# Hamedkiri/heuristique_style_transfer_code

Hardware: NVIDIA B200
Metric: images/sec (higher is better)
Workload: dtype tf32

## Files before the change

### heuristique_style_transfer_code_b200/_lib.py

```python
from __future__ import annotations

import ctypes
import os
from ctypes import c_int, c_longlong, c_void_p, POINTER, c_uint

from .build import LIB_PATH

_LIB = None

GH_DTYPE_F32 = 0
GH_DTYPE_BF16 = 1
GH_ERR_BAD_ARG = -1
GH_ERR_UNSUPPORTED = -2

_P = c_void_p
_SIGNATURES = {
    "gh_version": (c_int, []),
    "gh_sm_count": (c_int, []),
    "gh_set_option": (c_int, [ctypes.c_char_p, c_int]),
    "gh_last_device_error": (c_int, [POINTER(c_uint)]),
    "gh_gram_pool_fwd": (c_int, [_P, c_int, c_longlong, c_longlong, c_longlong, c_int, c_int, c_int, c_int, _P, c_int,
                                  c_int, c_int, c_int, _P]),
    "gh_gram_dense_fwd": (c_int, [_P, c_int, c_longlong, c_longlong, c_longlong, c_int, c_int, c_int, _P, c_int, c_int,
                                   _P]),
    "gh_adaptive_pool_fwd": (c_int, [_P, c_int, c_int, c_int, _P, c_int, c_int, _P]),
    "gh_adaptive_pool_bwd": (c_int, [_P, c_int, c_int, c_int, c_int, c_int, _P, _P]),
    "gh_gram_pool_bwd": (c_int, [_P, c_int, c_longlong, c_longlong, c_longlong, c_int, c_int, c_int, c_int, _P, c_int,
                                  c_int, _P, c_int, c_longlong, c_longlong, c_longlong, c_int, _P]),
    "gh_gram_dense_bwd": (c_int, [_P, c_int, c_longlong, c_longlong, c_longlong, c_int, c_int, c_int, _P, _P, c_int,
                                   c_longlong, c_longlong, c_longlong, c_int, _P]),
    "gh_attn_head_fwd": (c_int, [_P] * 7 + [c_int] * 4 + [_P] * 5 + [_P]),
    "gh_transpose_cast": (c_int, [_P, c_int, _P, c_int, c_int, c_int, c_int, c_longlong, _P]),
    "gh_preprocess_frame": (c_int, [_P, c_longlong, c_int, c_int, c_int, _P, _P, _P, c_int, _P, _P, _P, c_int, _P, _P, _P,
                                     c_int, c_int, _P]),
    "gh_normalize_u8": (c_int, [_P, _P, c_longlong, c_int, c_longlong, _P, _P, _P]),
    "gh_gemm_f32": (c_int, [_P, c_longlong, c_longlong, _P, c_longlong, c_longlong, _P, _P, c_longlong, c_int, c_int,
                             c_int, _P]),
    "gh_maxpool2d_nhwc": (c_int, [_P, c_int, _P] + [c_int] * 7 + [_P]),
    "gh_stem_space_to_depth": (c_int, [_P] + [c_longlong] * 4 + [c_int] * 3 + [_P, c_int, _P]),
    "gh_patch_gram_workspace": (c_longlong, [c_int, c_int, c_int]),
    "gh_patch_gram_fwd": (c_int, [_P, _P, _P, _P, c_int, c_int, c_int, c_int, _P, _P, _P, _P]),
    "gh_patch_attn_fwd": (c_int, [_P] * 11 + [c_int] * 5 + [_P, _P, _P]),
    "gh_attn_head_bwd_workspace": (c_longlong, [c_int, c_int, c_int]),
    "gh_attn_head_bwd": (c_int, [_P] * 10 + [c_int] * 4 + [_P] * 8 + [_P]),
    "gh_gram_mse_blocks": (c_int, [c_longlong]),
    "gh_gram_mse": (c_int, [_P, _P, c_longlong, _P, _P, _P]),
    "gh_split_bf16": (c_int, [_P, _P, c_longlong, c_longlong, _P]),
    "gh_gemm_planes": (c_int, [_P, c_longlong, c_longlong, c_int, _P, c_longlong, c_longlong, c_int, _P, _P, _P,
                                c_longlong, c_longlong, c_int, c_int, c_int, c_int, _P]),
    "gh_tgemm_plan": (c_int, [c_int, c_int, c_int, c_int, c_int, POINTER(c_int), POINTER(c_int), POINTER(c_int)]),
    "gh_gram_bwd_plan": (c_int, [c_int, c_int, c_int, c_int, c_int, POINTER(c_int)]),
    "gh_attn_head_fwd2": (c_int, [_P] * 7 + [c_int] * 4 + [_P] * 6 + [_P]),
    "gh_attn_head_bwd2_workspace": (c_longlong, [c_int, c_int, c_int]),
    "gh_attn_head_bwd2": (c_int, [_P] * 10 + [c_int] * 4 + [_P] * 8 + [_P]),
}
EXPORTED_SYMBOLS = tuple(_SIGNATURES)


class GramHeadError(RuntimeError):
    pass


def library_path() -> str:
    return os.environ.get("GRAMHEAD_LIB", LIB_PATH)


def lib() -> ctypes.CDLL:
    global _LIB
    if _LIB is None:
        path = library_path()
        if not os.path.isfile(path):
            raise GramHeadError(
# ... 43 lines not shown
```

### heuristique_style_transfer_code_b200/build.py

```python
from __future__ import annotations

import os
import shutil
import subprocess

CSRC = os.path.join(os.path.dirname(os.path.abspath(__file__)), "csrc")
LIB_PATH = os.path.join(CSRC, "libgramhead.so")
SOURCES = ["gramhead.cu", "common.cuh", "gram_fwd.cuh", "pair.cuh", "gram_fwd_pair.cuh", "gram_bwd.cuh", "gram_bwd2.cuh", "gram_bwd_pair.cuh",
           "umma_gemm.cuh", "tgemm_pair.cuh", "launch.cuh", "attn_head.cuh", "attn_head2.cuh", "preprocess.cuh", "transpose.cuh", "patchgan.cuh", "pool.cuh", "style_loss.cuh"]
NVCC_FLAGS = ["-gencode", "arch=compute_100a,code=sm_100a", "-O3", "-lineinfo", "-std=c++17",
              "-Xcompiler", "-fPIC", "-shared"]


def _nvcc() -> str:
    for cand in (os.environ.get("NVCC"), shutil.which("nvcc"), "/usr/local/cuda/bin/nvcc"):
        if cand and os.path.isfile(cand):
            return cand
    raise RuntimeError("gramhead: nvcc not found (set NVCC=/path/to/nvcc)")


def is_stale() -> bool:
    if not os.path.isfile(LIB_PATH):
        return True
    built = os.path.getmtime(LIB_PATH)
    deps = [os.path.join(CSRC, s) for s in SOURCES]
    deps.append(os.path.join(os.path.dirname(os.path.dirname(CSRC)), "include", "gramhead.h"))
    return any(os.path.getmtime(d) > built for d in deps if os.path.isfile(d))


def build_library(force: bool = False, verbose: bool = False) -> str:
    if not force and not is_stale():
        return LIB_PATH
    cmd = [_nvcc(), *NVCC_FLAGS, "gramhead.cu", "-o", LIB_PATH + ".tmp"]
    if verbose:
        cmd.insert(1, "-Xptxas=-v")
    res = subprocess.run(cmd, cwd=CSRC, capture_output=True, text=True)
    if res.returncode != 0:
        raise RuntimeError("gramhead: nvcc failed\n" + res.stdout + res.stderr)
    if verbose:
        print(res.stderr)
    os.replace(LIB_PATH + ".tmp", LIB_PATH)
    return LIB_PATH
# ... 5 lines not shown
```

### heuristique_style_transfer_code_b200/csrc/common.cuh

```cuda
#pragma once
#include <cuda_runtime.h>
#include <cuda_bf16.h>
#include <stdint.h>

namespace gh {

__device__ unsigned int* g_dev_error_ptr = nullptr;

__device__ __forceinline__ void dev_fail(unsigned int code, unsigned int site) {
  unsigned int* rec = g_dev_error_ptr;
  if (rec != nullptr && atomicCAS_system(rec, 0u, code) == 0u) {
    rec[1] = blockIdx.x;
    rec[2] = threadIdx.x;
    rec[3] = site;
    __threadfence_system();
  }
  __trap();
}

inline volatile unsigned int* error_record_host() {
  static unsigned int* host_rec[64] = {nullptr};
  int dev = 0;
  if (cudaGetDevice(&dev) != cudaSuccess || dev < 0 || dev >= 64) return nullptr;
  if (host_rec[dev] == nullptr) {
// ... 130 lines not shown
      "{%0, %1, %2, %3, %4, %5, %6, %7, %8, %9, %10, %11, %12, %13, %14, %15, "
      "%16, %17, %18, %19, %20, %21, %22, %23, %24, %25, %26, %27, %28, %29, %30, %31}, [%32];"
      : "=r"(r[0]), "=r"(r[1]), "=r"(r[2]), "=r"(r[3]), "=r"(r[4]), "=r"(r[5]), "=r"(r[6]), "=r"(r[7]),
        "=r"(r[8]), "=r"(r[9]), "=r"(r[10]), "=r"(r[11]), "=r"(r[12]), "=r"(r[13]), "=r"(r[14]), "=r"(r[15]),
        "=r"(r[16]), "=r"(r[17]), "=r"(r[18]), "=r"(r[19]), "=r"(r[20]), "=r"(r[21]), "=r"(r[22]), "=r"(r[23]),
        "=r"(r[24]), "=r"(r[25]), "=r"(r[26]), "=r"(r[27]), "=r"(r[28]), "=r"(r[29]), "=r"(r[30]), "=r"(r[31])
      : "r"(taddr)
      : "memory");
}
__device__ __forceinline__ void tmem_ld_wait() { asm volatile("tcgen05.wait::ld.sync.aligned;" ::: "memory"); }

constexpr uint32_t kTileK = 64;
constexpr uint32_t kRowBytes = 128;
constexpr uint32_t kAtomBytes = 1024;
constexpr uint32_t kUmmaK = 16;

__host__ __device__ constexpr uint64_t make_smem_desc_sw128(uint32_t smem_addr) {
  return (uint64_t)((smem_addr & 0x3FFFFu) >> 4)
         | ((uint64_t)1 << 16)
         | ((uint64_t)(kAtomBytes >> 4) << 32)
         | ((uint64_t)1 << 46)
         | ((uint64_t)2 << 61);
}
__host__ __device__ constexpr uint32_t make_idesc_bf16(uint32_t m, uint32_t n) {
  return (1u << 4)
         | (1u << 7)
         | (1u << 10)
         | ((n >> 3) << 17)
         | ((m >> 4) << 24);
}
__device__ __forceinline__ uint32_t sw128_off(uint32_t r, uint32_t k) {
  return (r >> 3) * kAtomBytes + (r & 7u) * kRowBytes + ((((k >> 3) ^ r) & 7u) << 4) + ((k & 7u) << 1);
}

__device__ __forceinline__ float4 ldg_stream_f4(const float* p) {
  float4 v;
  asm volatile("ld.global.nc.L1::no_allocate.L2::128B.v4.f32 {%0, %1, %2, %3}, [%4];"
               : "=f"(v.x), "=f"(v.y), "=f"(v.z), "=f"(v.w)
               : "l"(p));
  return v;
}
__device__ __forceinline__ uint2 ldg_stream_u2(const void* p) {
  uint2 v;
  asm volatile("ld.global.nc.L1::no_allocate.v2.u32 {%0, %1}, [%2];" : "=r"(v.x), "=r"(v.y) : "l"(p));
  return v;
}
__device__ __forceinline__ void sts_u2(uint32_t addr, uint32_t a, uint32_t b) {
  asm volatile("st.shared.v2.b32 [%0], {%1, %2};" ::"r"(addr), "r"(a), "r"(b) : "memory");
}
__device__ __forceinline__ void sts_u4(uint32_t addr, uint32_t a, uint32_t b, uint32_t c, uint32_t d) {
  asm volatile("st.shared.v4.b32 [%0], {%1, %2, %3, %4};" ::"r"(addr), "r"(a), "r"(b), "r"(c), "r"(d) : "memory");
}
__device__ __forceinline__ uint32_t pack_bf16x2(float lo, float hi) {
  __nv_bfloat162 h = __floats2bfloat162_rn(lo, hi);
  return *reinterpret_cast<uint32_t*>(&h);
}
__device__ __forceinline__ void red_add_f32(float* p, float v) {
  asm volatile("red.global.add.f32 [%0], %1;" ::"l"(p), "f"(v) : "memory");
}

}
```

### heuristique_style_transfer_code_b200/csrc/gramhead.cu

```cuda
#include "../../include/gramhead.h"
#include "common.cuh"
#include "gram_fwd.cuh"
#include "gram_fwd_pair.cuh"
#include "gram_bwd.cuh"
#include "gram_bwd2.cuh"
#include "gram_bwd_pair.cuh"
#include "attn_head.cuh"
#include "umma_gemm.cuh"
#include "tgemm_pair.cuh"
#include "attn_head2.cuh"
#include "preprocess.cuh"
#include "transpose.cuh"
#include "patchgan.cuh"
#include "pool.cuh"
#include "style_loss.cuh"
#include <string>

namespace gh {

static int sm_count_cached() {
  static int cached[64] = {0};
  int dev = 0;
  if (cudaGetDevice(&dev) != cudaSuccess || dev < 0 || dev >= 64) return 148;
  if (cached[dev] == 0) {
    int n = 0;
    if (cudaDeviceGetAttribute(&n, cudaDevAttrMultiProcessorCount, dev) != cudaSuccess || n <= 0) n = 148;
    cached[dev] = n;
    error_record_host();
  }
  return cached[dev];
}

static int ilog2_exact(int v) {
  if (v <= 0 || (v & (v - 1))) return -1;
  int s = 0;
  while ((1 << s) < v) ++s;
  return s;
}

static int choose_ksplit(long long base_units, int nkb, int ctas, bool balance = false) {
  if (base_units >= ctas) {
    if (!balance) return 1;
    const long long r1 = (base_units + ctas - 1) / ctas * 2, r2 = (2 * base_units + ctas - 1) / ctas;
    return (nkb >= 8 && r2 * 100 <= r1 * 93) ? 2 : 1;
  }
  long long ks = (2LL * ctas + base_units - 1) / base_units;
  const int kmax = nkb / 2 > 1 ? nkb / 2 : 1;
// ... 690 lines not shown
  MaxPoolParams p{};
  p.in = in; p.out = out; p.B = B; p.H = H; p.W = W; p.C = C; p.k = k; p.stride = stride; p.pad = pad;
  p.OH = (H + 2 * pad - k) / stride + 1;
  p.OW = (W + 2 * pad - k) / stride + 1;
  if (p.OH <= 0 || p.OW <= 0) return GH_ERR_BAD_ARG;
  p.total_vec = (long long)B * p.OH * p.OW * (C / vec);
  const int cv = C / vec;
  if (cv > 256 || B > 65535) return GH_ERR_UNSUPPORTED;
  const int ppc = 256 / cv;
  const dim3 grid((p.OW + ppc - 1) / ppc, (p.OH + kPoolRows - 1) / kPoolRows, B);
  if (grid.y > 65535) return GH_ERR_UNSUPPORTED;
  if (dtype == GH_DTYPE_F32) maxpool2d_nhwc_kernel<float><<<grid, 256, 0, (cudaStream_t)stream>>>(p);
  else maxpool2d_nhwc_kernel<__nv_bfloat16><<<grid, 256, 0, (cudaStream_t)stream>>>(p);
  return (int)cudaGetLastError();
}

int gh_stem_space_to_depth(const float* x, long long img_stride, long long c_stride, long long y_stride,
                           long long x_stride, int B, int H, int W, void* z, int z_dtype, void* stream) {
  if (!x || !z || B <= 0 || H <= 0 || W <= 0) return GH_ERR_BAD_ARG;
  if (z_dtype != GH_DTYPE_F32 && z_dtype != GH_DTYPE_BF16) return GH_ERR_BAD_ARG;
  if ((H & 1) || (W & 1) || (uintptr_t)z % 16 != 0) return GH_ERR_UNSUPPORTED;
  StemS2DParams p{};
  p.x = x; p.z = z; p.s_img = img_stride; p.s_c = c_stride; p.s_y = y_stride; p.s_x = x_stride;
  p.B = B; p.H = H; p.W = W; p.HP = H / 2 + 3; p.WP = W / 2 + 3;
  p.total = (long long)B * p.HP * p.WP;
  const long long want = (p.total + 255) / 256;
  const long long cap = (long long)gh_sm_count() * 32;
  const int grid = (int)(want < cap ? want : cap);
  if (z_dtype == GH_DTYPE_F32) stem_space_to_depth_kernel<float><<<grid, 256, 0, (cudaStream_t)stream>>>(p);
  else stem_space_to_depth_kernel<__nv_bfloat16><<<grid, 256, 0, (cudaStream_t)stream>>>(p);
  return (int)cudaGetLastError();
}

int gh_gram_mse_blocks(long long n) {
  if (n <= 0) return 0;
  long long blocks = (n / 4 + kMseThreads - 1) / kMseThreads;
  const long long cap = (long long)sm_count_cached() * 4 < kMseMaxBlocks ? (long long)sm_count_cached() * 4 : kMseMaxBlocks;
  if (blocks > cap) blocks = cap;
  return (int)(blocks < 1 ? 1 : blocks);
}

int gh_gram_mse(const float* G, const float* G_target, long long n, float* dG, float* partial, void* stream) {
  if (!G || !G_target || !dG || !partial || n <= 0) return GH_ERR_BAD_ARG;
  if (n % 4 != 0 || ((uintptr_t)G | (uintptr_t)G_target | (uintptr_t)dG) % 16 != 0) return GH_ERR_UNSUPPORTED;
  gram_mse_kernel<<<gh_gram_mse_blocks(n), kMseThreads, 0, (cudaStream_t)stream>>>(G, G_target, dG, partial, n / 4,
                                                                                   1.0f / (float)n);
  return (int)cudaGetLastError();
}

long long gh_patch_gram_workspace(int L, int B, int D) {
  if (L <= 0 || B <= 0 || D <= 0) return 0;
  return (long long)L * B * D * (kPatchBins + 4);
}

int gh_patch_gram_fwd(const float* const* maps, const int* H, const int* W, const long long* strides, int L, int B,
                      int D, int ln_input, float* gram, float* gram_norm, float* workspace, void* stream) {
  if (!maps || !H || !W || !strides || !gram || !gram_norm || !workspace || L <= 0 || B <= 0 || D <= 0)
    return GH_ERR_BAD_ARG;
  if ((uintptr_t)workspace % 8 != 0) return GH_ERR_BAD_ARG;
  if (L > kPatchMaxLayers || D > kPatchMaxD || B > 0x7fffffff / 2) return GH_ERR_UNSUPPORTED;
  PatchGramParams p{};
  for (int l = 0; l < L; ++l) {
    if (!maps[l] || H[l] <= 0 || W[l] <= 0) return GH_ERR_BAD_ARG;
    p.layer[l].x = maps[l];
    p.layer[l].H = H[l];
    p.layer[l].W = W[l];
// ... 260 lines not shown
```

### heuristique_style_transfer_code_b200/frozen_encoder.py

```python
from __future__ import annotations

import os
from typing import List, Optional, Tuple

import torch
import torch.nn as nn
import torch.nn.functional as F

from . import ops

STEM_SPACE_TO_DEPTH = os.environ.get("GRAMHEAD_STEM_S2D", "1") != "0"


def _stem_space_to_depth_weight(weight: torch.Tensor) -> torch.Tensor:
    o = weight.shape[0]
    w8 = weight.new_zeros((o, 3, 8, 8))
    w8[:, :, 1:, 1:] = weight
    w12 = w8.view(o, 3, 4, 2, 4, 2).permute(0, 1, 3, 5, 2, 4).reshape(o, 12, 4, 4)
    w16 = weight.new_zeros((o, 16, 4, 4))
    w16[:, :12] = w12
    return w16.contiguous(memory_format=torch.channels_last)


def _fold(conv: nn.Conv2d, bn: nn.BatchNorm2d, dtype: torch.dtype, channels_last: bool):
    var, mean = bn.running_var.detach().float(), bn.running_mean.detach().float()
    gamma = bn.weight.detach().float() if bn.weight is not None else torch.ones_like(var)
    beta = bn.bias.detach().float() if bn.bias is not None else torch.zeros_like(var)
    scale = gamma * torch.rsqrt(var + bn.eps)
    weight = conv.weight.detach().float() * scale.view(-1, 1, 1, 1)
    bias = beta - mean * scale
    if conv.bias is not None:
        bias = bias + conv.bias.detach().float() * scale
    weight = weight.to(dtype).contiguous(memory_format=torch.channels_last if channels_last else torch.contiguous_format)
    return weight, bias.to(dtype).contiguous(), conv.stride, conv.padding, conv.dilation, conv.groups


def _foldable(conv, bn) -> bool:
    return (isinstance(conv, nn.Conv2d) and type(bn) is nn.BatchNorm2d and bn.track_running_stats
            and bn.running_mean is not None and bn.running_var is not None and conv.padding_mode == "zeros"
            and not isinstance(conv.padding, str))


def _is_bottleneck(block) -> bool:
    names = ("conv1", "bn1", "conv2", "bn2", "conv3", "bn3", "relu", "downsample")
    if type(block).__name__ != "Bottleneck" or not all(hasattr(block, n) for n in names):
        return False
    if not isinstance(block.relu, nn.ReLU):
        return False
    ok = _foldable(block.conv1, block.bn1) and _foldable(block.conv2, block.bn2) and _foldable(block.conv3, block.bn3)
    if block.downsample is not None:
        ds = block.downsample
        ok = ok and isinstance(ds, nn.Sequential) and len(ds) == 2 and _foldable(ds[0], ds[1])
    return ok


def encoder_signature(encoder: nn.Module) -> Optional[Tuple]:
    try:
        return tuple((t.data_ptr(), t._version) for t in list(encoder.parameters()) + list(encoder.buffers()))
    except RuntimeError:
        return None


class FoldedEncoder:

    def __init__(self, stem, pool, stages, signature, dtype, channels_last):
        self.stem, self.pool, self.stages = stem, pool, stages
        self.stem_s2d = None
        self.signature, self.dtype, self.channels_last = signature, dtype, channels_last

    @staticmethod
    def supported(encoder: nn.Sequential) -> bool:
        if len(encoder) < 4:
            return False
        if not (_foldable(encoder[0], encoder[1]) and isinstance(encoder[2], nn.ReLU) and isinstance(encoder[3], nn.MaxPool2d)):
            return False
        for stage in list(encoder)[4:]:
            if not isinstance(stage, nn.Sequential) or not all(_is_bottleneck(b) for b in stage):
                return False
        return True

    @classmethod
    def build(cls, encoder: nn.Sequential, dtype: torch.dtype, channels_last: bool) -> Optional["FoldedEncoder"]:
        if not cls.supported(encoder):
            return None
        with torch.no_grad():
            stem = _fold(encoder[0], encoder[1], dtype, channels_last)
            conv1 = encoder[0]
            stem_s2d = None
            if (STEM_SPACE_TO_DEPTH and channels_last and conv1.in_channels == 3 and conv1.kernel_size == (7, 7)
                    and conv1.stride == (2, 2) and conv1.padding == (3, 3) and conv1.dilation == (1, 1) and conv1.groups == 1):
                stem_s2d = (_stem_space_to_depth_weight(stem[0].float()).to(dtype), stem[1], (1, 1), (0, 0), (1, 1), 1)
            stages: List[list] = []
            for stage in list(encoder)[4:]:
                blocks = []
                for b in stage:
                    c3 = _fold(b.conv3, b.bn3, dtype, channels_last)
                    down = None
                    if b.downsample is not None:
                        dw, db, *geom = _fold(b.downsample[0], b.downsample[1], torch.float32, channels_last)
                        bias3 = (c3[1].float() + db).to(dtype)
                        c3 = (c3[0], bias3) + tuple(c3[2:])
                        down = (dw.to(dtype).contiguous(memory_format=torch.channels_last if channels_last
                                                        else torch.contiguous_format), None) + tuple(geom)
                    blocks.append((_fold(b.conv1, b.bn1, dtype, channels_last), _fold(b.conv2, b.bn2, dtype, channels_last),
                                   c3, down))
                stages.append(blocks)
        plan = cls(stem, encoder[3], stages, encoder_signature(encoder), dtype, channels_last)
        plan.stem_s2d = stem_s2d
        return plan

    @staticmethod
    def _conv_relu(x, p):
        w, b, stride, padding, dilation, groups = p
        return torch.cudnn_convolution_relu(x, w, b, stride, padding, dilation, groups)

    def _pool(self, x):
        p = self.pool
        k, s, pad = p.kernel_size, p.stride, p.padding
        plain = (isinstance(k, int) and isinstance(s, int) and isinstance(pad, int) and p.dilation == 1
                 and not p.ceil_mode and not p.return_indices)
        vec = 4 if x.dtype == torch.float32 else 8
        if plain and self.channels_last and x.shape[1] % vec == 0 and x.is_contiguous(memory_format=torch.channels_last):
            return ops.maxpool2d_nhwc(x, k, s, pad)
        return p(x)

    def __call__(self, x: torch.Tensor):
        if (self.stem_s2d is not None and x.dtype == torch.float32 and x.shape[1] == 3 and x.shape[2] % 2 == 0
                and x.shape[3] % 2 == 0):
            x = self._conv_relu(ops.stem_space_to_depth(x, self.dtype), self.stem_s2d)
        else:
            x = x.to(self.dtype)
            if self.channels_last:
                x = x.contiguous(memory_format=torch.channels_last)
            x = self._conv_relu(x, self.stem)
        x = self._pool(x)
        outs = []
        for blocks in self.stages:
            for c1, c2, c3, down in blocks:
                identity = x
                y = self._conv_relu(x, c1)
                y = self._conv_relu(y, c2)
                if down is not None:
                    identity = F.conv2d(x, down[0], down[1], down[2], down[3], down[4], down[5])
                w, b, stride, padding, dilation, groups = c3
                x = torch.cudnn_convolution_add_relu(y, w, identity, 1.0, b, stride, padding, dilation, groups)
            outs.append(x)
        return x, outs
```

### heuristique_style_transfer_code_b200/ops.py

```python
from __future__ import annotations

import ctypes
from typing import List, Optional, Sequence, Tuple

import torch

from . import _lib
from ._lib import GH_DTYPE_BF16, GH_DTYPE_F32, GramHeadError, check

KSPLIT = 0
MAX_CTAS = 0

LAUNCHES = 0
PROFILE = None


class _Timed:
    def __init__(self, name, kernels, device, **work):
        self.name, self.kernels, self.device, self.work = name, kernels, device, work

    def __enter__(self):
        global LAUNCHES
        LAUNCHES += self.kernels
        if PROFILE is not None:
# ... 202 lines not shown
        rc = _lib.lib().gh_gemm_f32(a.data_ptr(), a.stride(0), a.stride(1), b.data_ptr(), b.stride(0), b.stride(1),
                                    0 if bias is None else bias.data_ptr(), out.data_ptr(), n, m, n, k, _stream_ptr(a))
    check(rc, "gh_gemm_f32")
    return out


def maxpool2d_nhwc(x: torch.Tensor, kernel: int, stride: int, padding: int) -> torch.Tensor:
    _require_cuda(x, "x")
    if x.dim() != 4 or not x.is_contiguous(memory_format=torch.channels_last):
        raise GramHeadError("gramhead: maxpool2d_nhwc takes a channels_last (B, C, H, W) tensor")
    b, c, h, w = x.shape
    oh, ow = (h + 2 * padding - kernel) // stride + 1, (w + 2 * padding - kernel) // stride + 1
    out = torch.empty((b, c, oh, ow), device=x.device, dtype=x.dtype, memory_format=torch.channels_last)
    work = dict(bytes=(x.numel() + out.numel()) * x.element_size(), flops=0, kind="maxpool")
    with torch.cuda.device(x.device), _Timed(f"maxpool2d_nhwc[C={c},HW={h}x{w},{x.dtype}]", 1, x.device, **work):
        rc = _lib.lib().gh_maxpool2d_nhwc(x.data_ptr(), _dtype_code(x), out.data_ptr(), b, h, w, c, kernel, stride, padding,
                                          _stream_ptr(x))
    check(rc, "gh_maxpool2d_nhwc")
    return out


def stem_space_to_depth(x: torch.Tensor, dtype: torch.dtype) -> torch.Tensor:
    _require_cuda(x, "x")
    if x.dim() != 4 or x.shape[1] != 3 or x.dtype != torch.float32 or x.shape[2] % 2 or x.shape[3] % 2:
        raise GramHeadError("gramhead: stem_space_to_depth takes fp32 (B, 3, H, W) images with even H and W")
    b, _, h, w = x.shape
    z = torch.empty((b, 16, h // 2 + 3, w // 2 + 3), device=x.device, dtype=dtype, memory_format=torch.channels_last)
    work = dict(bytes=x.numel() * 4 + z.numel() * z.element_size(), flops=0, kind="stem_s2d")
    with torch.cuda.device(x.device), _Timed(f"stem_space_to_depth[HW={h}x{w},{dtype}]", 1, x.device, **work):
        rc = _lib.lib().gh_stem_space_to_depth(x.data_ptr(), x.stride(0), x.stride(1), x.stride(2), x.stride(3), b, h, w,
                                               z.data_ptr(), _dtype_code(z), _stream_ptr(x))
    check(rc, "gh_stem_space_to_depth")
    return z


def normalize_u8(x: torch.Tensor, mean, std, out: Optional[torch.Tensor] = None) -> torch.Tensor:
    _require_cuda(x, "x")
    if x.dim() != 4 or x.dtype != torch.uint8 or not 1 <= x.shape[1] <= 4:
        raise GramHeadError("gramhead: normalize_u8 takes a (B, C <= 4, H, W) uint8 batch")
    mean, std = [float(v) for v in mean], [float(v) for v in std]
    b, c, h, w = x.shape
    if len(mean) != c or len(std) != c:
        raise GramHeadError(f"gramhead: normalize_u8: {c} channels need {c} means and stds")
    x = x.contiguous()
    if out is None:
        out = torch.empty((b, c, h, w), device=x.device, dtype=torch.float32)
    else:
        if (out.dtype != torch.float32 or out.device != x.device or out.dim() != 4 or out.shape[0] < b
                or out.shape[1:] != x.shape[1:] or not out.is_contiguous()):
            raise GramHeadError("gramhead: normalize_u8: `out` must be a dense fp32 (>= B, C, H, W) tensor on x's device")
        out = out[:b]
    if b == 0:
        return out
    fl = ctypes.c_float * c
    work = dict(bytes=x.numel() * 5, flops=0, kind="normalize_u8")
    with torch.cuda.device(x.device), _Timed(f"normalize_u8[C={c},HW={h}x{w}]", 1, x.device, **work):
        rc = _lib.lib().gh_normalize_u8(x.data_ptr(), out.data_ptr(), b, c, h * w, fl(*mean), fl(*std), _stream_ptr(x))
    check(rc, "gh_normalize_u8")
    return out


def patch_gram(maps: Sequence[torch.Tensor], ln_input: bool = True):
    import ctypes
    L = len(maps)
    if L == 0:
        raise GramHeadError("gramhead: patch_gram needs at least one feature map")
# ... 337 lines not shown
```

### include/gramhead.h

```cpp
#ifndef GRAMHEAD_H_
#define GRAMHEAD_H_

#ifdef __cplusplus
extern "C" {
#endif

#define GH_ERR_BAD_ARG (-1)
#define GH_ERR_UNSUPPORTED (-2)

#define GH_DTYPE_F32 0
#define GH_DTYPE_BF16 1

int gh_version(void);

int gh_sm_count(void);

int gh_set_option(const char* name, int value);

int gh_last_device_error(unsigned int* out4);

int gh_gram_pool_fwd(const void* F, int f_dtype, long long img_stride, long long row_stride, long long x_stride, int B,
                     int C, int HW, int g, float* desc, int l, int L, int ksplit, int max_ctas, void* stream);

int gh_gram_dense_fwd(const void* F, int f_dtype, long long img_stride, long long row_stride, long long x_stride, int B,
// ... 4 lines not shown

int gh_gram_pool_bwd(const void* F, int f_dtype, long long img_stride, long long row_stride, long long x_stride, int B,
                     int C, int HW, int g, const float* d_desc, int l, int L, void* dF, int df_dtype,
                     long long df_img_stride, long long df_row_stride, long long df_x_stride, int max_ctas, void* stream);

int gh_gram_dense_bwd(const void* F, int f_dtype, long long img_stride, long long row_stride, long long x_stride, int B,
                      int C, int HW, const float* dG, void* dF, int df_dtype, long long df_img_stride,
                      long long df_row_stride, long long df_x_stride, int max_ctas, void* stream);

int gh_attn_head_fwd(const float* desc, const float* W_in, const float* b_in, const float* W_out, const float* b_out,
                     const float* W_c, const float* b_c, int B, int L, int E, int nc, float* qkv, float* probs,
                     float* obar, float* emb, float* logits, void* stream);

int gh_transpose_cast(const void* in, int in_dtype, void* out, int out_dtype, int B, int R, int S, long long out_pitch,
                      void* stream);

int gh_preprocess_frame(const unsigned char* frame, long long pitch_bytes, int H, int W, int bgr, const int* hx_min,
                        const int* hx_size, const int* hk, int hkmax, const int* vy_min, const int* vy_size, const int* vk,
                        int vkmax, const float* mean3_host, const float* std3_host, float* out, int OH, int OW,
                        void* stream);

int gh_normalize_u8(const unsigned char* src, float* dst, long long images, int channels, long long hw,
                    const float* mean_host, const float* std_host, void* stream);

int gh_gemm_f32(const float* A, long long a_sm, long long a_sk, const float* B, long long b_sk, long long b_sn,
                const float* bias, float* D, long long ldd, int M, int N, int K, void* stream);

int gh_maxpool2d_nhwc(const void* in, int dtype, void* out, int B, int H, int W, int C, int k, int stride, int pad,
                      void* stream);

int gh_stem_space_to_depth(const float* x, long long img_stride, long long c_stride, long long y_stride,
                           long long x_stride, int B, int H, int W, void* z, int z_dtype, void* stream);

long long gh_patch_gram_workspace(int L, int B, int D);
int gh_patch_gram_fwd(const float* const* maps, const int* H, const int* W, const long long* strides, int L, int B,
                      int D, int ln_input, float* gram, float* gram_norm, float* workspace, void* stream);

int gh_patch_attn_fwd(const float* feat, const float* W_in1, const float* b_in1, const float* W_out1,
                      const float* b_out1, const float* W_in2, const float* b_in2, const float* W_out2,
                      const float* b_out2, const float* W_c, const float* b_c, int L, int B, int E, int heads, int nc,
                      float* emb, float* logits, void* stream);

long long gh_attn_head_bwd_workspace(int B, int L, int E);

int gh_attn_head_bwd(const float* desc, const float* W_in, const float* W_out, const float* W_c, const float* qkv,
                     const float* probs, const float* obar, const float* emb, const float* d_logits,
                     const float* d_emb_ext, int B, int L, int E, int nc, float* d_desc, float* dW_in, float* db_in,
                     float* dW_out, float* db_out, float* dW_c, float* db_c, float* workspace, void* stream);

int gh_gram_mse_blocks(long long n);
int gh_gram_mse(const float* G, const float* G_target, long long n, float* dG, float* partial, void* stream);

int gh_split_bf16(const float* src, void* planes, long long n, long long plane_stride, void* stream);

int gh_gemm_planes(const void* A_planes, long long lda, long long a_plane_stride, int a_mn, const void* B_planes,
                   long long ldb, long long b_plane_stride, int b_mn, const float* bias, float* D, void* D_planes,
                   long long ldd, long long d_plane_stride, int M, int N, int K, int max_split, void* stream);

int gh_tgemm_plan(int M, int N, int K, int max_split, int npairs, int* tn, int* ksplit, int* units);

int gh_gram_bwd_plan(int C, int HW, int g, int f_dtype, int channels_last, int* out);

int gh_attn_head_fwd2(const float* desc, const void* w_in_planes, const float* b_in, const void* w_out_planes,
                      const float* b_out, const float* W_c, const float* b_c, int B, int L, int E, int nc, void* x_planes,
                      float* qkv, float* probs, void* obar_planes, float* emb, float* logits, void* stream);

// ... 13 lines not shown
```

Baseline: 41410.

## Fuse stem conv, bias, ReLU and maxpool into one warp-specialized tcgen05 kernel

Adds a persistent warp-specialized kernel that does the ResNet stem in one pass. Producer warps load raw NCHW pixels straight into space-to-depth TF32 tiles in shared memory, and an MMA warp issues tcgen05 TF32 UMMAs into tensor memory. Epilogue warps then max-reduce three conv rows and neighbouring columns, add the bias, apply ReLU and write the pooled NHWC output. This removes the separate space-to-depth, conv and maxpool launches and their intermediate activation round trips through global memory. The cost is a complex mbarrier pipeline, a halo recomputation across tiles, and TF32 rounding of the stem, gated on allow_tf32.

```diff
diff --git a/heuristique_style_transfer_code_b200/_lib.py b/heuristique_style_transfer_code_b200/_lib.py
--- a/heuristique_style_transfer_code_b200/_lib.py
+++ b/heuristique_style_transfer_code_b200/_lib.py
@@ -38,6 +38,7 @@
                              c_int, _P]),
     "gh_maxpool2d_nhwc": (c_int, [_P, c_int, _P] + [c_int] * 7 + [_P]),
     "gh_stem_space_to_depth": (c_int, [_P] + [c_longlong] * 4 + [c_int] * 3 + [_P, c_int, _P]),
+    "gh_stem_conv_pool_nhwc": (c_int, [_P] + [c_longlong] * 4 + [c_int] * 3 + [_P] * 4),
     "gh_patch_gram_workspace": (c_longlong, [c_int, c_int, c_int]),
     "gh_patch_gram_fwd": (c_int, [_P, _P, _P, _P, c_int, c_int, c_int, c_int, _P, _P, _P, _P]),
     "gh_patch_attn_fwd": (c_int, [_P] * 11 + [c_int] * 5 + [_P, _P, _P]),
diff --git a/heuristique_style_transfer_code_b200/build.py b/heuristique_style_transfer_code_b200/build.py
--- a/heuristique_style_transfer_code_b200/build.py
+++ b/heuristique_style_transfer_code_b200/build.py
@@ -7,7 +7,7 @@
 CSRC = os.path.join(os.path.dirname(os.path.abspath(__file__)), "csrc")
 LIB_PATH = os.path.join(CSRC, "libgramhead.so")
 SOURCES = ["gramhead.cu", "common.cuh", "gram_fwd.cuh", "pair.cuh", "gram_fwd_pair.cuh", "gram_bwd.cuh", "gram_bwd2.cuh", "gram_bwd_pair.cuh",
-           "umma_gemm.cuh", "tgemm_pair.cuh", "launch.cuh", "attn_head.cuh", "attn_head2.cuh", "preprocess.cuh", "transpose.cuh", "patchgan.cuh", "pool.cuh", "style_loss.cuh"]
+           "umma_gemm.cuh", "tgemm_pair.cuh", "launch.cuh", "attn_head.cuh", "attn_head2.cuh", "preprocess.cuh", "transpose.cuh", "patchgan.cuh", "pool.cuh", "stem.cuh", "style_loss.cuh"]
 NVCC_FLAGS = ["-gencode", "arch=compute_100a,code=sm_100a", "-O3", "-lineinfo", "-std=c++17",
               "-Xcompiler", "-fPIC", "-shared"]
 
diff --git a/heuristique_style_transfer_code_b200/csrc/common.cuh b/heuristique_style_transfer_code_b200/csrc/common.cuh
--- a/heuristique_style_transfer_code_b200/csrc/common.cuh
+++ b/heuristique_style_transfer_code_b200/csrc/common.cuh
@@ -186,6 +186,29 @@
 __device__ __forceinline__ uint32_t sw128_off(uint32_t r, uint32_t k) {
   return (r >> 3) * kAtomBytes + (r & 7u) * kRowBytes + ((((k >> 3) ^ r) & 7u) << 4) + ((k & 7u) << 1);
 }
+__host__ __device__ constexpr uint32_t make_idesc_tf32(uint32_t m, uint32_t n) {
+  return (1u << 4) | (2u << 7) | (2u << 10) | ((n >> 3) << 17) | ((m >> 4) << 24);
+}
+__host__ __device__ constexpr uint64_t make_smem_desc_noswz(uint32_t addr, uint32_t lbo, uint32_t sbo) {
+  return (uint64_t)((addr & 0x3FFFFu) >> 4) | ((uint64_t)((lbo >> 4) & 0x3FFFu) << 16) |
+         ((uint64_t)((sbo >> 4) & 0x3FFFu) << 32) | ((uint64_t)1 << 46);
+}
+__device__ __forceinline__ void umma_tf32(uint32_t tmem_d, uint64_t desc_a, uint64_t desc_b, uint32_t idesc,
+                                          uint32_t accumulate) {
+  asm volatile(
+      "{\n\t"
+      ".reg .pred p;\n\t"
+      "setp.ne.b32 p, %4, 0;\n\t"
+      "tcgen05.mma.cta_group::1.kind::tf32 [%0], %1, %2, %3, p;\n\t"
+      "}\n" ::"r"(tmem_d),
+      "l"(desc_a), "l"(desc_b), "r"(idesc), "r"(accumulate)
+      : "memory");
+}
+__device__ __forceinline__ uint32_t tf32_rna(float f) {
+  uint32_t r;
+  asm("cvt.rna.tf32.f32 %0, %1;" : "=r"(r) : "f"(f));
+  return r;
+}
 
 __device__ __forceinline__ float4 ldg_stream_f4(const float* p) {
   float4 v;
diff --git a/heuristique_style_transfer_code_b200/csrc/gramhead.cu b/heuristique_style_transfer_code_b200/csrc/gramhead.cu
--- a/heuristique_style_transfer_code_b200/csrc/gramhead.cu
+++ b/heuristique_style_transfer_code_b200/csrc/gramhead.cu
@@ -13,6 +13,7 @@
 #include "transpose.cuh"
 #include "patchgan.cuh"
 #include "pool.cuh"
+#include "stem.cuh"
 #include "style_loss.cuh"
 #include <string>
 
@@ -769,6 +770,29 @@
   return (int)cudaGetLastError();
 }
 
+int gh_stem_conv_pool_nhwc(const float* x, long long img_stride, long long c_stride, long long y_stride,
+                           long long x_stride, int B, int H, int W, const float* w_packed, const float* bias, float* out,
+                           void* stream) {
+  if (!x || !w_packed || !bias || !out || B <= 0 || H <= 0 || W <= 0) return GH_ERR_BAD_ARG;
+  if ((H & 1) || (W & 1) || (uintptr_t)w_packed % 16 != 0 || (uintptr_t)out % 16 != 0) return GH_ERR_UNSUPPORTED;
+  StemConvPoolParams p{};
+  p.x = x; p.s_img = img_stride; p.s_c = c_stride; p.s_y = y_stride; p.s_x = x_stride;
+  p.w = w_packed; p.bias = bias; p.out = out;
+  p.B = B; p.OH = H / 2; p.OW = W / 2;
+  p.PH = (p.OH - 1) / 2 + 1;
+  p.PW = (p.OW - 1) / 2 + 1;
+  p.tiles = (p.PW + kScTileCols - 1) / kScTileCols;
+  p.vec2 = x_stride == 1 && (uintptr_t)x % 8 == 0 && (img_stride % 2 == 0) && (c_stride % 2 == 0) && (y_stride % 2 == 0);
+  p.units = (long long)B * p.tiles * p.PH;
+  const int sms = sm_count_cached();
+  const int grid = (int)(p.units < sms ? p.units : sms);
+  cudaError_t e = cudaFuncSetAttribute(stem_conv_pool_kernel, cudaFuncAttributeMaxDynamicSharedMemorySize,
+                                       (int)kScSmemBytes);
+  if (e != cudaSuccess) return (int)e;
+  stem_conv_pool_kernel<<<grid, kScThreads, kScSmemBytes, (cudaStream_t)stream>>>(p);
+  return (int)cudaGetLastError();
+}
+
 int gh_gram_mse_blocks(long long n) {
   if (n <= 0) return 0;
   long long blocks = (n / 4 + kMseThreads - 1) / kMseThreads;
diff --git a/heuristique_style_transfer_code_b200/csrc/stem.cuh b/heuristique_style_transfer_code_b200/csrc/stem.cuh
--- /dev/null
+++ b/heuristique_style_transfer_code_b200/csrc/stem.cuh
@@ -0,0 +1,281 @@
+#pragma once
+#include "common.cuh"
+
+namespace gh {
+
+constexpr int kScProducerWarps = 8;
+constexpr int kScEpiWarp0 = 8;
+constexpr int kScMmaWarp = 12;
+constexpr int kScThreads = 13 * 32;
+constexpr int kScTileCols = 63;
+constexpr int kScCells = 131;
+constexpr int kScItems = 3 * kScCells;
+constexpr int kScItemIters = (kScItems + 31) / 32;
+constexpr int kScSlots = 12;
+constexpr int kScAccSlots = 8;
+constexpr uint32_t kScSlotBytes = kScCells * 16;
+constexpr uint32_t kScPlaneBytes = kScSlots * kScSlotBytes;
+constexpr uint32_t kScWBytes = 16 * 2 * 2048;
+constexpr uint32_t kScAOff = kScWBytes;
+constexpr uint32_t kScBiasOff = kScAOff + 4 * kScPlaneBytes;
+constexpr uint32_t kScXbufOff = kScBiasOff + 64 * 4;
+constexpr uint32_t kScBarOff = kScXbufOff + 2 * 4 * 64 * 4;
+constexpr uint32_t kScBarBytes = 8 * (2 * kScSlots + 2 * kScAccSlots) + 16;
+constexpr uint32_t kScSmemBytes = kScBarOff + kScBarBytes + 1024;
+
+struct StemConvPoolParams {
+  const float* x;
+  long long s_img, s_c, s_y, s_x;
+  const float* w;
+  const float* bias;
+  float* out;
+  int B, OH, OW, PH, PW, tiles;
+  int vec2;
+  long long units;
+};
+
+__device__ __forceinline__ float max_nan(float a, float b) { return (b > a || b != b) ? b : a; }
+
+struct ScSeg {
+  int b, j, py0, py1, y_lo, y_hi;
+};
+__device__ __forceinline__ bool sc_next(const StemConvPoolParams& p, long long& u, long long u1, ScSeg& s) {
+  if (u >= u1) return false;
+  const long long bj = u / p.PH;
+  const long long end = (bj + 1) * p.PH < u1 ? (bj + 1) * p.PH : u1;
+  s.b = (int)(bj / p.tiles);
+  s.j = (int)(bj - (long long)s.b * p.tiles);
+  s.py0 = (int)(u - bj * p.PH);
+  s.py1 = s.py0 + (int)(end - u);
+  s.y_lo = 2 * s.py0 - 1 > 0 ? 2 * s.py0 - 1 : 0;
+  s.y_hi = 2 * s.py1 - 1 < p.OH - 1 ? 2 * s.py1 - 1 : p.OH - 1;
+  u = end;
+  return true;
+}
+
+__global__ void __launch_bounds__(kScThreads, 1) stem_conv_pool_kernel(const StemConvPoolParams p) {
+  extern __shared__ uint8_t smem_raw[];
+  const uint32_t raw = smem_u32(smem_raw);
+  const uint32_t base = (raw + 1023u) & ~1023u;
+  uint8_t* gbase = smem_raw + (base - raw);
+  const uint32_t w_smem = base, a_smem = base + kScAOff;
+  const float* bias_s = reinterpret_cast<const float*>(gbase + kScBiasOff);
+  float* xbuf = reinterpret_cast<float*>(gbase + kScXbufOff);
+  const uint32_t bar_full = base + kScBarOff, bar_empty = bar_full + 8 * kScSlots;
+  const uint32_t bar_afull = bar_empty + 8 * kScSlots, bar_aempty = bar_afull + 8 * kScAccSlots;
+  const uint32_t tmem_slot = bar_aempty + 8 * kScAccSlots;
+  volatile uint32_t* tmem_slot_ptr = reinterpret_cast<volatile uint32_t*>(gbase + (tmem_slot - base));
+  const int warp = threadIdx.x >> 5, lane = threadIdx.x & 31;
+
+  {
+    const float4* wg = reinterpret_cast<const float4*>(p.w);
+    float4* ws = reinterpret_cast<float4*>(gbase);
+    for (int i = threadIdx.x; i < (int)(kScWBytes / 16); i += kScThreads) ws[i] = __ldg(wg + i);
+    if (threadIdx.x < 64) reinterpret_cast<float*>(gbase + kScBiasOff)[threadIdx.x] = __ldg(p.bias + threadIdx.x);
+    float4* z = reinterpret_cast<float4*>(gbase + kScAOff + 3 * kScPlaneBytes);
+    for (int i = threadIdx.x; i < (int)(kScPlaneBytes / 16); i += kScThreads) z[i] = make_float4(0.f, 0.f, 0.f, 0.f);
+    fence_proxy_async_smem();
+  }
+  if (threadIdx.x == 0) {
+    for (int s = 0; s < kScSlots; ++s) {
+      mbar_init(bar_full + 8 * s, 1);
+      mbar_init(bar_empty + 8 * s, 1);
+    }
+    for (int s = 0; s < kScAccSlots; ++s) {
+      mbar_init(bar_afull + 8 * s, 1);
+      mbar_init(bar_aempty + 8 * s, 4);
+    }
+    mbar_fence_init();
+  }
+  if (warp == kScMmaWarp) tmem_alloc(tmem_slot, 512);
+  tc_fence_before_sync();
+  __syncthreads();
+  tc_fence_after_sync();
+  const uint32_t tmem_base = *tmem_slot_ptr;
+
+  const long long u0 = p.units * blockIdx.x / gridDim.x, u1 = p.units * (blockIdx.x + 1) / gridDim.x;
+
+  if (warp < kScProducerWarps) {
+    uint32_t gs = 0;
+    long long u = u0;
+    ScSeg sg;
+    while (sc_next(p, u, u1, sg)) {
+      const int n_stage = sg.y_hi - sg.y_lo + 4;
+      const float* img = p.x + (long long)sg.b * p.s_img;
+      for (int k = 0; k < n_stage; ++k) {
+        const uint32_t g = gs + (uint32_t)k;
+        if ((int)(g % kScProducerWarps) != warp) continue;
+        const uint32_t slot = g % kScSlots;
+        const int Y = sg.y_lo + k - 2;
+        const bool row_ok = Y >= 0 && Y < p.OH;
+        float4 v[kScItemIters];
+#pragma unroll
+        for (int it = 0; it < kScItemIters; ++it) {
+          const int i = it * 32 + lane;
+          const int c = i / kScCells, s = i - c * kScCells;
+          const int X = kScTileCols * 2 * sg.j + s - 3;
+          v[it] = make_float4(0.f, 0.f, 0.f, 0.f);
+          if (i < kScItems && row_ok && X >= 0 && X < p.OW) {
+            const float* q = img + (long long)c * p.s_c + (long long)(2 * Y) * p.s_y + (long long)(2 * X) * p.s_x;
+            if (p.vec2) {
+              const float2 t0 = __ldg(reinterpret_cast<const float2*>(q));
+              const float2 t1 = __ldg(reinterpret_cast<const float2*>(q + p.s_y));
+              v[it] = make_float4(t0.x, t0.y, t1.x, t1.y);
+            } else {
+              v[it] = make_float4(__ldg(q), __ldg(q + p.s_x), __ldg(q + p.s_y), __ldg(q + p.s_y + p.s_x));
+            }
+          }
+        }
+        mbar_wait(bar_empty + 8 * slot, ((g / kScSlots) & 1u) ^ 1u, 300u + slot);
+#pragma unroll
+        for (int it = 0; it < kScItemIters; ++it) {
+          const int i = it * 32 + lane;
+          if (i < kScItems) {
+            const int c = i / kScCells, s = i - c * kScCells;
+            sts_u4(a_smem + (uint32_t)c * kScPlaneBytes + slot * kScSlotBytes + (uint32_t)s * 16u, tf32_rna(v[it].x),
+                   tf32_rna(v[it].y), tf32_rna(v[it].z), tf32_rna(v[it].w));
+          }
+        }
+        fence_proxy_async_smem();
+        __syncwarp();
+        if (lane == 0) mbar_arrive(bar_full + 8 * slot);
+      }
+      gs += (uint32_t)n_stage;
+    }
+  } else if (warp == kScMmaWarp) {
+    constexpr uint32_t idesc = make_idesc_tf32(128, 64);
+    const uint64_t adesc0 = make_smem_desc_noswz(a_smem, kScPlaneBytes, 128);
+    const uint64_t bdesc0 = make_smem_desc_noswz(w_smem, 1024, 128);
+    uint32_t gs = 0, gc = 0;
+    long long u = u0;
+    ScSeg sg;
+    while (sc_next(p, u, u1, sg)) {
+      const int n_conv = sg.y_hi - sg.y_lo + 1;
+      for (int k = 0; k < n_conv; ++k, ++gc) {
+        const uint32_t acc = gc % kScAccSlots;
+        mbar_wait(bar_aempty + 8 * acc, ((gc / kScAccSlots) & 1u) ^ 1u, 400u + acc);
+        uint32_t slot[4];
+#pragma unroll
+        for (int a = 0; a < 4; ++a) {
+          const uint32_t g = gs + (uint32_t)(k + a);
+          slot[a] = g % kScSlots;
+          mbar_wait(bar_full + 8 * slot[a], (g / kScSlots) & 1u, 500u + slot[a]);
+        }
+        tc_fence_after_sync();
+        if (elect_one()) {
+          const uint32_t d = tmem_base + acc * 64u;
+#pragma unroll
+          for (int a = 0; a < 4; ++a) {
+            const uint64_t arow = adesc0 + ((slot[a] * kScSlotBytes) >> 4);
+#pragma unroll
+            for (int b = 0; b < 4; ++b)
+#pragma unroll
+              for (int h = 0; h < 2; ++h) {
+                const uint64_t da = arow + ((b * 16 + h * 2 * kScPlaneBytes) >> 4);
+                const uint64_t db = bdesc0 + ((((a * 4 + b) * 2 + h) * 2048) >> 4);
+                umma_tf32(d, da, db, idesc, (a | b | h) != 0);
+              }
+          }
+          umma_commit(bar_afull + 8 * acc);
+          umma_commit(bar_empty + 8 * slot[0]);
+          if (k == n_conv - 1)
+            for (int a = 1; a < 4; ++a) umma_commit(bar_empty + 8 * slot[a]);
+        }
+        __syncwarp();
+      }
+      gs += (uint32_t)(n_conv + 3);
+    }
+  } else {
+    const int quad = warp - kScEpiWarp0;
+    const uint32_t tlane = tmem_base + ((uint32_t)(32 * quad) << 16);
+    const float neg_inf = -__int_as_float(0x7f800000);
+    uint32_t gc = 0, xb = 0;
+    long long u = u0;
+    ScSeg sg;
+    while (sc_next(p, u, u1, sg)) {
+      const int x = kScTileCols * 2 * sg.j - 1 + 32 * quad + lane;
+      const bool col_ok = x >= 0 && x < p.OW;
+      auto acc_of = [&](int y) { return (gc + (uint32_t)(y - sg.y_lo)) % kScAccSlots; };
+      auto wait_row = [&](int y) {
+        const uint32_t g = gc + (uint32_t)(y - sg.y_lo);
+        mbar_wait(bar_afull + 8 * (g % kScAccSlots), (g / kScAccSlots) & 1u, 600u + g % kScAccSlots);
+      };
+      for (int py = sg.py0; py < sg.py1; ++py) {
+        const int ya = 2 * py - 1, yb = 2 * py, yc = 2 * py + 1;
+        const bool ha = ya >= sg.y_lo, hc = yc <= sg.y_hi;
+        if (py == sg.py0 && ha) wait_row(ya);
+        wait_row(yb);
+        if (hc) wait_row(yc);
+        tc_fence_after_sync();
+        float m[64];
+#pragma unroll
+        for (int h = 0; h < 2; ++h) {
+          uint32_t r[32];
+          tmem_ld32_nowait(tlane + acc_of(yb) * 64u + 32u * h, r);
+          tmem_ld_wait();
+#pragma unroll
+          for (int i = 0; i < 32; ++i) m[32 * h + i] = __uint_as_float(r[i]);
+          if (ha) {
+            tmem_ld32_nowait(tlane + acc_of(ya) * 64u + 32u * h, r);
+            tmem_ld_wait();
+#pragma unroll
+            for (int i = 0; i < 32; ++i) m[32 * h + i] = max_nan(m[32 * h + i], __uint_as_float(r[i]));
+          }
+          if (hc) {
+            tmem_ld32_nowait(tlane + acc_of(yc) * 64u + 32u * h, r);
+            tmem_ld_wait();
+#pragma unroll
+            for (int i = 0; i < 32; ++i) m[32 * h + i] = max_nan(m[32 * h + i], __uint_as_float(r[i]));
+          }
+        }
+        tc_fence_before_sync();
+        __syncwarp();
+        if (lane == 0) {
+          if (ha) mbar_arrive(bar_aempty + 8 * acc_of(ya));
+          mbar_arrive(bar_aempty + 8 * acc_of(yb));
+          if (hc && py == sg.py1 - 1) mbar_arrive(bar_aempty + 8 * acc_of(yc));
+        }
+        if (!col_ok) {
+#pragma unroll
+          for (int i = 0; i < 64; ++i) m[i] = neg_inf;
+        }
+        float* xs = xbuf + xb * 256;
+        if (lane == 0 && quad > 0) {
+#pragma unroll
+          for (int i = 0; i < 64; i += 4)
+            *reinterpret_cast<float4*>(xs + quad * 64 + i) = make_float4(m[i], m[i + 1], m[i + 2], m[i + 3]);
+        }
+        asm volatile("bar.sync 1, 128;" ::: "memory");
+        const bool from_next = lane == 30 && quad < 3;
+        const int qx = 16 * quad + (lane >> 1);
+        const int px = kScTileCols * sg.j + qx;
+        const bool store = !(lane & 1) && qx < kScTileCols && px < p.PW;
+        float4* o = reinterpret_cast<float4*>(p.out + (((long long)sg.b * p.PH + py) * p.PW + px) * 64);
+#pragma unroll
+        for (int i = 0; i < 64; i += 4) {
+          float r4[4];
+#pragma unroll
+          for (int e = 0; e < 4; ++e) {
+            const float v1 = __shfl_down_sync(0xffffffffu, m[i + e], 1);
+            float v2 = __shfl_down_sync(0xffffffffu, m[i + e], 2);
+            if (from_next) v2 = xs[(quad + 1) * 64 + i + e];
+            float t = max_nan(max_nan(m[i + e], v1), v2) + bias_s[i + e];
+            r4[e] = t != t ? t : fmaxf(t, 0.f);
+          }
+          if (store) o[i / 4] = make_float4(r4[0], r4[1], r4[2], r4[3]);
+        }
+        xb ^= 1u;
+      }
+      gc += (uint32_t)(sg.y_hi - sg.y_lo + 1);
+    }
+  }
+
+  tc_fence_before_sync();
+  __syncthreads();
+  if (warp == kScMmaWarp) {
+    tc_fence_after_sync();
+    tmem_dealloc(tmem_base, 512);
+  }
+}
+
+}
diff --git a/heuristique_style_transfer_code_b200/frozen_encoder.py b/heuristique_style_transfer_code_b200/frozen_encoder.py
--- a/heuristique_style_transfer_code_b200/frozen_encoder.py
+++ b/heuristique_style_transfer_code_b200/frozen_encoder.py
@@ -20,6 +20,17 @@
     w16 = weight.new_zeros((o, 16, 4, 4))
     w16[:, :12] = w12
     return w16.contiguous(memory_format=torch.channels_last)
+
+
+def _tf32_round(x: torch.Tensor) -> torch.Tensor:
+    bits = (x.contiguous().view(torch.int32).to(torch.int64) & 0xFFFFFFFF) + 0x1000
+    bits = bits & 0xFFFFE000
+    return torch.where(bits >= 2 ** 31, bits - 2 ** 32, bits).to(torch.int32).view(torch.float32)
+
+
+def pack_stem_weight(w16: torch.Tensor) -> torch.Tensor:
+    w = _tf32_round(w16.float().contiguous())
+    return w.view(64, 2, 2, 4, 4, 4).permute(4, 5, 1, 2, 0, 3).contiguous().view(-1)
 
 
 def _fold(conv: nn.Conv2d, bn: nn.BatchNorm2d, dtype: torch.dtype, channels_last: bool):
@@ -66,6 +77,8 @@
     def __init__(self, stem, pool, stages, signature, dtype, channels_last):
         self.stem, self.pool, self.stages = stem, pool, stages
         self.stem_s2d = None
+        self.stem_packed = None
+        self._stem_fused = True
         self.signature, self.dtype, self.channels_last = signature, dtype, channels_last
 
     @staticmethod
@@ -107,6 +120,11 @@
                 stages.append(blocks)
         plan = cls(stem, encoder[3], stages, encoder_signature(encoder), dtype, channels_last)
         plan.stem_s2d = stem_s2d
+        pool = encoder[3]
+        if (stem_s2d is not None and dtype == torch.float32 and conv1.out_channels == 64
+                and pool.kernel_size in (3, (3, 3)) and pool.stride in (2, (2, 2)) and pool.padding in (1, (1, 1))
+                and pool.dilation in (1, (1, 1)) and not pool.ceil_mode and not pool.return_indices):
+            plan.stem_packed = pack_stem_weight(stem_s2d[0])
         return plan
 
     @staticmethod
@@ -124,7 +142,11 @@
             return ops.maxpool2d_nhwc(x, k, s, pad)
         return p(x)
 
-    def __call__(self, x: torch.Tensor):
+    def stem_forward(self, x: torch.Tensor) -> torch.Tensor:
+        if (self.stem_packed is not None and self._stem_fused and torch.backends.cudnn.allow_tf32
+                and x.dtype == torch.float32 and x.dim() == 4 and x.shape[1] == 3 and x.shape[2] % 2 == 0
+                and x.shape[3] % 2 == 0):
+            return ops.stem_conv_pool(x, self.stem_packed, self.stem_s2d[1])
         if (self.stem_s2d is not None and x.dtype == torch.float32 and x.shape[1] == 3 and x.shape[2] % 2 == 0
                 and x.shape[3] % 2 == 0):
             x = self._conv_relu(ops.stem_space_to_depth(x, self.dtype), self.stem_s2d)
@@ -133,7 +155,10 @@
             if self.channels_last:
                 x = x.contiguous(memory_format=torch.channels_last)
             x = self._conv_relu(x, self.stem)
-        x = self._pool(x)
+        return self._pool(x)
+
+    def __call__(self, x: torch.Tensor):
+        x = self.stem_forward(x)
         outs = []
         for blocks in self.stages:
             for c1, c2, c3, down in blocks:
diff --git a/heuristique_style_transfer_code_b200/ops.py b/heuristique_style_transfer_code_b200/ops.py
--- a/heuristique_style_transfer_code_b200/ops.py
+++ b/heuristique_style_transfer_code_b200/ops.py
@@ -258,6 +258,26 @@
                                                z.data_ptr(), _dtype_code(z), _stream_ptr(x))
     check(rc, "gh_stem_space_to_depth")
     return z
+
+
+def stem_conv_pool(x: torch.Tensor, packed_weight: torch.Tensor, bias: torch.Tensor) -> torch.Tensor:
+    _require_cuda(x, "x")
+    if x.dim() != 4 or x.shape[1] != 3 or x.dtype != torch.float32 or x.shape[2] % 2 or x.shape[3] % 2:
+        raise GramHeadError("gramhead: stem_conv_pool takes fp32 (B, 3, H, W) images with even H and W")
+    if (packed_weight.dtype != torch.float32 or packed_weight.numel() != 16384 or not packed_weight.is_contiguous()
+            or bias.dtype != torch.float32 or bias.numel() != 64 or not bias.is_contiguous()
+            or packed_weight.device != x.device or bias.device != x.device):
+        raise GramHeadError("gramhead: stem_conv_pool takes the packed fp32 stem weights (16384) and bias (64) on x's device")
+    b, _, h, w = x.shape
+    oh, ow = h // 2, w // 2
+    ph, pw = (oh - 1) // 2 + 1, (ow - 1) // 2 + 1
+    out = torch.empty((b, 64, ph, pw), device=x.device, dtype=torch.float32, memory_format=torch.channels_last)
+    work = dict(bytes=(x.numel() + out.numel()) * 4, flops=2 * b * oh * ow * 64 * 147, kind="stem_conv_pool")
+    with torch.cuda.device(x.device), _Timed(f"stem_conv_pool[HW={h}x{w}]", 1, x.device, **work):
+        rc = _lib.lib().gh_stem_conv_pool_nhwc(x.data_ptr(), x.stride(0), x.stride(1), x.stride(2), x.stride(3), b, h, w,
+                                               packed_weight.data_ptr(), bias.data_ptr(), out.data_ptr(), _stream_ptr(x))
+    check(rc, "gh_stem_conv_pool_nhwc")
+    return out
 
 
 def normalize_u8(x: torch.Tensor, mean, std, out: Optional[torch.Tensor] = None) -> torch.Tensor:
diff --git a/include/gramhead.h b/include/gramhead.h
--- a/include/gramhead.h
+++ b/include/gramhead.h
@@ -60,6 +60,10 @@
 int gh_stem_space_to_depth(const float* x, long long img_stride, long long c_stride, long long y_stride,
                            long long x_stride, int B, int H, int W, void* z, int z_dtype, void* stream);
 
+int gh_stem_conv_pool_nhwc(const float* x, long long img_stride, long long c_stride, long long y_stride,
+                           long long x_stride, int B, int H, int W, const float* w_packed, const float* bias, float* out,
+                           void* stream);
+
 long long gh_patch_gram_workspace(int L, int B, int D);
 int gh_patch_gram_fwd(const float* const* maps, const int* H, const int* W, const long long* strides, int L, int B,
                       int D, int ln_input, float* gram, float* gram_norm, float* workspace, void* stream);
diff --git a/oracle/stem_fp64.py b/oracle/stem_fp64.py
--- /dev/null
+++ b/oracle/stem_fp64.py
@@ -0,0 +1,33 @@
+from __future__ import annotations
+
+import numpy as np
+
+from .head_fp64 import tf32_round
+
+
+def stem_fp64(x: np.ndarray, w: np.ndarray, bias: np.ndarray, round_operands: bool = True) -> np.ndarray:
+    x = np.asarray(x, dtype=np.float32)
+    w = np.asarray(w, dtype=np.float32)
+    if round_operands:
+        x, w = tf32_round(x), tf32_round(w)
+    x, w = x.astype(np.float64), w.astype(np.float64)
+    b, c, h, wd = x.shape
+    o = w.shape[0]
+    oh, ow = (h + 6 - 7) // 2 + 1, (wd + 6 - 7) // 2 + 1
+    xp = np.zeros((b, c, h + 6, wd + 6))
+    xp[:, :, 3:h + 3, 3:wd + 3] = x
+    conv = np.zeros((b, o, oh, ow))
+    for i in range(7):
+        for j in range(7):
+            patch = xp[:, :, i:i + 2 * oh:2, j:j + 2 * ow:2]
+            conv += np.einsum("bchw,oc->bohw", patch, w[:, :, i, j])
+    conv += np.asarray(bias, dtype=np.float64).reshape(1, o, 1, 1)
+    act = np.where(np.isnan(conv), conv, np.maximum(conv, 0.0))
+    ph, pw = (oh + 2 - 3) // 2 + 1, (ow + 2 - 3) // 2 + 1
+    ap = np.full((b, o, oh + 2, ow + 2), -np.inf)
+    ap[:, :, 1:oh + 1, 1:ow + 1] = act
+    out = np.full((b, o, ph, pw), -np.inf)
+    for i in range(3):
+        for j in range(3):
+            out = np.maximum(out, ap[:, :, i:i + 2 * ph:2, j:j + 2 * pw:2])
+    return out
```

New measurement: 44360, median of 6. +7.1%, better.
